# wtsi-svi/ReadServer

Hardware: AMD Instinct MI355X
Metric: 31-mer backward-search queries/sec on popBWT, counted as (query x shard) backward searches/s (higher is better)
Workload: dtype u64

## Files before the change

### readserver_amd/csrc/search_lines.hip

```cpp
#include <hip/hip_runtime.h>
#include <stdint.h>
#include <stdlib.h>
#include <string.h>

#include "kernels.h"
#include "line_format.h"
#include "rank_device.h"
#include "wave_lines.h"

namespace rsb {


__device__ __forceinline__ ulonglong2 start_record(const shard_view &ix, const uint64_t *pq, uint32_t k) {
    ulonglong2 rec;
    const uint64_t last = pq[(k - 1u) >> 5];
    if (view_uses_ktab(ix, k)) {
        const uint32_t T = ix.ktab_depth;
        const uint32_t off = 2u * (k - T);
        const uint32_t w0 = off >> 6, sh = off & 63u;
        uint64_t bits = (w0 == ((k - 1u) >> 5) ? last : pq[w0]) >> sh;
        if (sh + 2u * T > 64u) bits |= last << (64u - sh);
        const uint64_t e = ktab_entry(ix.ktab, ix.ktab_fmt, T, ix.ktab_stride, bits & ((1ull << (2u * T)) - 1ull));
        const uint32_t width = (uint32_t)(e >> COUNT_BITS);
        if (width != KTAB_WIDE && (e & COUNT_MASK) + width <= ix.n) {
// ... 101 lines not shown
    const uint32_t t = threadIdx.x;
    {
        const uint32_t v = t / nshards, s = t - v * nshards;
        if (v < V) {
            const shard_view &ix = shards[s];
            const bool tab = view_uses_ktab(ix, k);
            const uint32_t T = ix.ktab_depth, off = tab ? 2u * (k - T) : 0u;
            const uint64_t *ktab = ix.ktab;
            const uint32_t fmt = ix.ktab_fmt, stride = ix.ktab_stride;
            const uint64_t n = ix.n;
            uint8_t ok[INIT_U];
            uint64_t word[INIT_U], e[INIT_U];
#pragma unroll
            for (uint32_t u = 0; u < INIT_U; ++u) {
                const size_t q = q0 + (size_t)u * V + v;
                const bool in = q < Q;
                ok[u] = in ? valid[q] : (uint8_t)2;
                word[u] = in ? packed[q] : 0ull;
            }
#pragma unroll
            for (uint32_t u = 0; u < INIT_U; ++u)
                e[u] = (tab && ok[u] == 1) ? ktab_entry(ktab, fmt, T, stride, (word[u] >> off) & ((1ull << (2u * T)) - 1ull)) : ~0ull;
#pragma unroll
            for (uint32_t u = 0; u < INIT_U; ++u) {
                if (ok[u] == 2) continue;
                ulonglong2 rec;
                const uint32_t width = (uint32_t)(e[u] >> COUNT_BITS);
                if (ok[u] == 0) {
                    rec.x = INIT_INVALID;
                    rec.y = 0;
                } else if (tab && width != KTAB_WIDE && (e[u] & COUNT_MASK) + width <= n) {
                    rec.x = e[u] & COUNT_MASK;
                    rec.y = rec.x + width - 1ull;
                } else {
                    const uint32_t b = (uint32_t)((word[u] >> (2u * ((k - 1u) & 31u))) & 3u) + 1u;
                    rec.x = ix.C[b] | INIT_FALLBACK;
                    rec.y = ix.C[b] + ix.total[b] - 1ull;
                }
                tile[u][v * nshards + s] = rec;
            }
        }
    }
    __syncthreads();
    {
        const uint32_t s = t / V, v = t - s * V;
        if (s < nshards) {
#pragma unroll
            for (uint32_t u = 0; u < INIT_U; ++u) {
                const size_t q = q0 + (size_t)u * V + v;
                if (q < Q) init[(size_t)s * Q + q] = tile[u][v * nshards + s];
            }
        }
    }
}

__global__ void __launch_bounds__(256)
search_init_1mm_kernel(const shard_view *__restrict__ shards, uint32_t nshards, const uint64_t *__restrict__ vpacked,
                       const uint8_t *__restrict__ vvalid, size_t mv, uint32_t k, uint32_t wpq, uint32_t V,
                       const ulonglong2 *__restrict__ trace, uint32_t trace_n,
                       ulonglong2 *__restrict__ init) {
    const size_t t_ = (size_t)blockIdx.x * blockDim.x + threadIdx.x;
    if (t_ >= mv * nshards) return;
    const size_t i = t_ / nshards, s = t_ - i * nshards;
    ulonglong2 rec;
    if (vvalid[i] == 0) {
        rec.x = INIT_INVALID;
        rec.y = 0;
    } else {
        const size_t q = i / V;
        const uint32_t v = (uint32_t)(i - q * V);
        const uint32_t pos = v ? (v - 1u) / 3u : ~0u;
        if (pos < trace_n) {
            const ulonglong2 t = trace[(s * (mv / V) + q) * trace_n + pos];
            rec.x = (t.x & COUNT_MASK) | ((uint64_t)pos << COUNT_BITS) | INIT_EXPLICIT;
            rec.y = t.y;
        } else {
            rec = start_record(shards[s], vpacked + i * wpq, k);
        }
    }
    init[s * mv + i] = rec;
}

enum { WORK_STEPS = 0, WORK_OCC = 1, WORK_LINES = 2, WORK_KTAB = 3, WORK_PHASE0 = 4, WORK_PASSES = 10, WORK_HOPS = 11, WORK_SOLO = 12 };

template <bool COUNT_WORK, bool COUNTS_ONLY, bool LONGK, int ROLE>
__global__ void __launch_bounds__(64 * WG_WAVES, RSB_MIN_WGS_PER_CU)
search_lines_kernel(const shard_view *__restrict__ shards, uint32_t nshards, const uint64_t *__restrict__ packed,
                    const ulonglong2 *__restrict__ init, unsigned long long *__restrict__ next_query,
                    size_t Q, uint32_t k, uint32_t wpq,
                    uint64_t *__restrict__ out_lower, uint64_t *__restrict__ out_upper,
                    unsigned long long *__restrict__ work,
                    ulonglong2 *__restrict__ trace, uint32_t trace_n, uint32_t qchunk, uint32_t pairs) {
    __shared__ uint4 s_stage[WG_WAVES][64 * SLOT_U4];
    const uint32_t lane = threadIdx.x & 63u;
    const uint32_t wave = threadIdx.x >> 6;
    const uint32_t side = lane >> 5;
    uint4 *stage = s_stage[wave];
    const uint32_t stage_lds = __builtin_amdgcn_readfirstlane((uint32_t)(uintptr_t)(lds_void_ptr)stage);
    const uint32_t swz = lane & 7u;
    const lds_u32 *own_row = reinterpret_cast<const lds_u32 *>(stage + (lane & 7u) * 64u + (lane >> 3) * SLOT_U4);
#define MINE(d) (mine0 + (((((uint32_t)(d)) >> 2) ^ swz) << 2) + (((uint32_t)(d)) & 3u))

    unsigned long long w_steps = 0, w_occ = 0, w_lines = 0, w_hops = 0, w_ktab = 0;
    unsigned long long ph[6] = {0, 0, 0, 0, 0, 0}, stamp = 0, passes = 0;
#define STAMP(i)                                                        \
    if (COUNT_WORK) {                                                   \
        __builtin_amdgcn_sched_barrier(0);                              \
        const unsigned long long now_ = __builtin_amdgcn_s_memtime();   \
        asm volatile("s_waitcnt lgkmcnt(0)" ::: "memory");              \
        ph[i] += now_ - stamp;                                          \
        stamp = now_;                                                   \
        __builtin_amdgcn_sched_barrier(0);                              \
    }
    if (COUNT_WORK) stamp = __builtin_amdgcn_s_memtime();

    uint32_t sid = blockIdx.x % nshards;
    for (uint32_t visited = 0; visited < nshards; ++visited, sid = (sid + 1u == nshards) ? 0u : sid + 1u) {
        const shard_view *sv = shards + sid;
        const char *lines_bytes = reinterpret_cast<const char *>(sv->lines);
        const uint32_t S = sv->sp.S;
        const double inv = sv->sp.inv;
        const uint32_t nlines = (uint32_t)sv->nlines;
        const bool ktab = view_uses_ktab(*sv, k);
        const int j_table = ktab ? (int)(k - sv->ktab_depth) - 1 : (int)k - 2;
        const uint32_t w_table = j_table > 0 ? (uint32_t)j_table >> 5 : 0u;
        const ulonglong2 *init_s = init + (size_t)sid * Q;
        uint64_t *out_lo = out_lower + (size_t)sid * Q * (pairs ? 2u : 1u);
        uint64_t *out_up = (COUNTS_ONLY || pairs) ? nullptr : out_upper + (size_t)sid * Q;
        unsigned long long *pool = next_query + (size_t)sid * POOL_STRIDE;
        if (visited != 0u && __hip_atomic_load(pool, __ATOMIC_RELAXED, __HIP_MEMORY_SCOPE_AGENT) >= (unsigned long long)Q) continue;
        ulonglong2 *trace_s = trace ? trace + (size_t)sid * Q * trace_n : nullptr;
        unsigned long long *hit_map = pairs == 2u ? reinterpret_cast<unsigned long long *>(out_upper) + (size_t)sid * hit_map_words(Q) : nullptr;
        uint32_t ctab_lo, ctab_hi;
        {
            const uint64_t c1 = sv->C[1], c2 = sv->C[2], c3 = sv->C[3], c4 = sv->C[4];
            const uint32_t l3 = lane & 3u;
            const uint64_t cv = l3 == 0u ? c1 : l3 == 1u ? c2 : l3 == 2u ? c3 : c4;
            ctab_lo = (uint32_t)cv;
            ctab_hi = (uint32_t)(cv >> 32);
        }

        const uint32_t QCHUNK = qchunk;
        uint64_t pool_next = 0, pool_end = 0;
        bool drained = false;
        size_t q = 0;
        bool has_q = false;
        size_t nq = 0;
        bool has_n = false;
        ulonglong2 nrec = {0, 0};
        uint64_t nword = 0;
        int j = 0;
        uint64_t word = 0, lo = 0, hi = 0;
        bool ready = false;
        uint64_t occ_hold = 0, cacc = 0;
        uint32_t cont = 0, cblk = 0, cdw = 0, co = 0, tries = 0;

        for (;;) {
            bool done = false;
            if (!has_q && has_n) {
                has_q = true;
                has_n = false;
                q = nq;
                if (nrec.x & INIT_INVALID) {
                    lo = 1;
                    hi = 0;
                    j = -1;
// ... 209 lines not shown
                const uint64_t occL = side ? other : occ_hold;
                const uint64_t occU = side ? occ_hold : other;
                if (COUNT_WORK && side == 0u) w_steps += 1;
                lo = pb + occL;
                hi = pb + occU - 1ull;
                --j;
                done = (lo > hi) || (j < 0);
                ready = false;
            }
            if (got_n) {
                nrec = rec;
                nword = first_word;
                has_n = true;
            }
            if (alive && done) {
                if (trace && side == 0u) {
                    for (int jj = j < (int)trace_n ? j : (int)trace_n - 1; jj >= 0; --jj)
                        trace_s[q * trace_n + (uint32_t)jj] = make_ulonglong2(lo, hi);
                }
                if (side == 0u) {
                    if (COUNTS_ONLY) {
                        if (hi >= lo) out_lo[q] = hi - lo + 1ull;
                    } else if (pairs == 2u) {
                        if (lo <= hi) {
                            reinterpret_cast<ulonglong2 *>(out_lo)[q] = make_ulonglong2(lo, hi);
                            atomicOr(hit_map + (q >> 6), 1ull << (q & 63u));
                        }
                    } else if (pairs) {
#ifdef RSB_NT_RESULTS
                        __builtin_nontemporal_store(lo, &out_lo[2 * q]);
                        __builtin_nontemporal_store(hi, &out_lo[2 * q + 1]);
#else
                        reinterpret_cast<ulonglong2 *>(out_lo)[q] = make_ulonglong2(lo, hi);
#endif
                    } else {
                        out_lo[q] = lo;
                        out_up[q] = hi;
                    }
                }
                has_q = false;
            }
            STAMP(5)
            if (COUNT_WORK) ++passes;
        }
    }
    if (COUNT_WORK) {
        if (lane == 0u) {
            for (int i = 0; i < 6; ++i) atomicAdd(&work[WORK_PHASE0 + i], ph[i]);
            atomicAdd(&work[WORK_PASSES], passes);
        }
        if (w_steps) atomicAdd(&work[WORK_STEPS], w_steps);
        if (w_occ) atomicAdd(&work[WORK_OCC], w_occ);
        if (w_lines) atomicAdd(&work[WORK_LINES], w_lines);
        if (w_ktab) atomicAdd(&work[WORK_KTAB], w_ktab);
        if (w_hops) atomicAdd(&work[WORK_HOPS], w_hops);
    }
#undef MINE
#undef STAMP
}

}
#include "search_solo.h"
namespace rsb {

static int search_kernel_choice() {
    static const int choice = [] {
        const char *e = getenv("RSBWT_SEARCH_KERNEL");
        if (e && !strcmp(e, "pair")) return 0;
        if (e && !strcmp(e, "solo")) return 1;
        return 2;
    }();
    return choice;
}

template <bool CW, bool CO>
static void launch_solo(int grid, hipStream_t stream, const shard_view *shards, uint32_t nshards, const uint64_t *pk,
                        const ulonglong2 *init, const uint8_t *valid, unsigned long long *ctr, size_t Q, uint32_t k, uint32_t wpq,
                        uint64_t *lo, uint64_t *up, unsigned long long *work, ulonglong2 *trace, uint32_t trace_n,
                        uint32_t pairs, bool fused) {
    uint32_t qchunk = 1024;
    while (qchunk > 64u && (size_t)qchunk * (size_t)grid * WG_WAVES * 4u > Q * nshards) qchunk >>= 1;
    static const bool no_staged = getenv("RSBWT_NO_STAGED_RESULTS") != nullptr;
    const bool staged = !CO && pairs != 2u && !no_staged;
    const uint32_t pa = pairs | (staged ? SOLO_STAGED_RESULTS : 0u);
    const size_t dyn = staged ? SOLO_RESULTS_LDS : 0u;
    if (fused)
        hipLaunchKernelGGL((search_solo_kernel<CW, CO, false, true>), dim3(grid), dim3(64 * WG_WAVES), dyn, stream, shards, nshards,
                           pk, init, valid, ctr, Q, k, wpq, lo, up, work, trace, trace_n, qchunk, pa);
    else if (wpq > 1)
        hipLaunchKernelGGL((search_solo_kernel<CW, CO, true>), dim3(grid), dim3(64 * WG_WAVES), dyn, stream, shards, nshards,
                           pk, init, valid, ctr, Q, k, wpq, lo, up, work, trace, trace_n, qchunk, pa);
    else
        hipLaunchKernelGGL((search_solo_kernel<CW, CO, false>), dim3(grid), dim3(64 * WG_WAVES), dyn, stream, shards, nshards,
                           pk, init, valid, ctr, Q, k, wpq, lo, up, work, trace, trace_n, qchunk, pa);
}

template <bool CW, bool CO>
static void launch_k(int grid, hipStream_t stream, const shard_view *shards, uint32_t nshards, const uint64_t *pk,
                     const ulonglong2 *init, unsigned long long *ctr, size_t Q, uint32_t k, uint32_t wpq,
                     uint64_t *lo, uint64_t *up, unsigned long long *work, ulonglong2 *trace, uint32_t trace_n,
                     uint32_t pairs) {
    uint32_t qchunk = 1024;
    while (qchunk > 32u && (size_t)qchunk * (size_t)grid * WG_WAVES * 4u > Q * nshards) qchunk >>= 1;
    if (wpq > 1)
        hipLaunchKernelGGL((search_lines_kernel<CW, CO, true, 0>), dim3(grid), dim3(64 * WG_WAVES), 0, stream, shards, nshards,
                           pk, init, ctr, Q, k, wpq, lo, up, work, trace, trace_n, qchunk, pairs);
    else
        hipLaunchKernelGGL((search_lines_kernel<CW, CO, false, 0>), dim3(grid), dim3(64 * WG_WAVES), 0, stream, shards, nshards,
                           pk, init, ctr, Q, k, wpq, lo, up, work, trace, trace_n, qchunk, pairs);
}

static void launch_init(const shard_view *d_shards, uint32_t nshards, const uint64_t *pk, const uint8_t *vd, size_t Q, uint32_t k,
                        uint32_t wpq, ulonglong2 *init, hipStream_t stream) {
    static const bool untiled = getenv("RSBWT_INIT_UNTILED") != nullptr;
    static const bool one_per_thread = getenv("RSBWT_INIT_ONE_PER_THREAD") != nullptr;
    if (nshards >= 2u && nshards <= 256u && !untiled && wpq == 1u && !one_per_thread) {
        const uint32_t V = 256u / nshards;
        hipLaunchKernelGGL(search_init_tiled4_kernel, dim3((unsigned)((Q + (size_t)V * INIT_U - 1) / ((size_t)V * INIT_U))), dim3(256), 0, stream,
                           d_shards, nshards, pk, vd, Q, k, V, init);
    } else if (nshards >= 2u && nshards <= 256u && !untiled) {
        const uint32_t V = 256u / nshards;
        hipLaunchKernelGGL(search_init_tiled_kernel, dim3((unsigned)((Q + V - 1) / V)), dim3(256), 0, stream, d_shards, nshards, pk, vd, Q,
                           k, wpq, V, init);
    } else {
        const size_t nrec = Q * nshards;
        hipLaunchKernelGGL(search_init_kernel, dim3((unsigned)((nrec + 255) / 256)), dim3(256), 0, stream, d_shards, nshards, pk, vd, Q, k,
                           wpq, init);
    }
}

hipError_t launch_search_init_var(const shard_view *d_shards, uint32_t nshards, const void *d_packed, const void *d_valid,
                                  const void *d_len, size_t Q, uint32_t wpq, void *d_init, hipStream_t stream) {
    if (Q == 0 || nshards == 0) return hipSuccess;
    const size_t nrec = Q * nshards;
    hipLaunchKernelGGL(search_init_var_kernel, dim3((unsigned)((nrec + 255) / 256)), dim3(256), 0, stream, d_shards, nshards,
                       (const uint64_t *)d_packed, (const uint8_t *)d_valid, (const uint32_t *)d_len, Q, wpq, (ulonglong2 *)d_init);
    return hipGetLastError();
}

hipError_t launch_search_init(const shard_view *d_shards, uint32_t nshards, const void *d_packed, const void *d_valid, size_t Q,
                              uint32_t k, void *d_init, hipStream_t stream) {
    if (Q == 0 || nshards == 0) return hipSuccess;
    const uint32_t wpq = (k + 31u) / 32u ? (k + 31u) / 32u : 1u;
    launch_init(d_shards, nshards, (const uint64_t *)d_packed, (const uint8_t *)d_valid, Q, k, wpq, (ulonglong2 *)d_init, stream);
    return hipGetLastError();
}

hipError_t launch_search(scratch_cache &scratch, const shard_view *d_shards, uint32_t nshards, const void *d_packed,
                         const void *d_valid, size_t Q, uint32_t k, void *d_lower, void *d_upper, bool counts_only,
                         unsigned long long *d_work, int num_cus, hipStream_t stream, hipEvent_t ev0, hipEvent_t ev1,
                         const search_extra *extra) {
    if (Q == 0 || nshards == 0) return hipSuccess;
    if (extra && extra->table_build && nshards != 1) return hipErrorInvalidValue;
    const bool hit_list = extra && extra->d_hit_bits && !counts_only;
    const uint32_t pairs = hit_list ? 2u : (extra && extra->pairs && !counts_only) ? 1u : 0u;
    ulonglong2 *trace = extra ? (ulonglong2 *)extra->d_trace_out : nullptr;
    const uint32_t trace_n = extra ? extra->trace_n : 0u;
    const uint32_t wpq = (k + 31u) / 32u ? (k + 31u) / 32u : 1u;
    const bool table_build = extra && extra->table_build;
    const int choice = search_kernel_choice();
    size_t g = 0;
    static const int wgs_per_cu = [] {
        const char *e = getenv("RSBWT_WAVE_WGS_PER_CU");
        const int v = e ? atoi(e) : 0;
        return v > 0 ? v : RSB_MIN_WGS_PER_CU;
    }();
    static const size_t spare_wgs = [] {
// ... 183 lines not shown
```

### readserver_amd/csrc/search_solo.h

```cpp
#ifndef RSBWT_SEARCH_SOLO_H
#define RSBWT_SEARCH_SOLO_H

namespace rsb {

constexpr uint64_t WL_DEAD = 1ull << 63;
constexpr uint32_t SOLO_STAGED_RESULTS = 4u;
constexpr uint32_t SOLO_RESULTS_LDS = WG_WAVES * 2048u;
constexpr uint32_t RES_BUFS = 15u;

#ifndef RSB_WALK1MM_WGS_PER_CU
#define RSB_WALK1MM_WGS_PER_CU 3
#endif
template <bool COUNT_WORK, bool COUNTS_ONLY, bool LONGK, bool FUSED = false, bool WL = false, bool WALK = false>
__global__ void __launch_bounds__(64 * WG_WAVES, WALK ? RSB_WALK1MM_WGS_PER_CU : RSB_MIN_WGS_PER_CU)
search_solo_kernel(const shard_view *__restrict__ shards, uint32_t nshards, const uint64_t *__restrict__ packed,
                   const ulonglong2 *__restrict__ init, const uint8_t *__restrict__ valid,
                   unsigned long long *__restrict__ next_query,
                   size_t Q, uint32_t k, uint32_t wpq,
                   uint64_t *__restrict__ out_lower, uint64_t *__restrict__ out_upper,
                   unsigned long long *__restrict__ work,
                   ulonglong2 *__restrict__ trace, uint32_t trace_n, uint32_t qchunk, uint32_t pairs_arg,
                   const unsigned long long *__restrict__ wl_counts = nullptr, size_t wl_cap = 0, size_t wl_implicit = 0) {
    __shared__ uint4 s_stage[WG_WAVES][64 * SLOT_U4];
    extern __shared__ uint4 s_results[];
    const uint32_t lane = threadIdx.x & 63u;
    const uint32_t wave = threadIdx.x >> 6;
    uint4 *stage = s_stage[wave];
    const uint32_t stage_lds = __builtin_amdgcn_readfirstlane((uint32_t)(uintptr_t)(lds_void_ptr)stage);
    const uint32_t swz = lane & 7u;
    const uint32_t pairs = pairs_arg & 3u;
    constexpr bool CAN_STAGE = !COUNTS_ONLY && !WL && !WALK;
    const bool stage_out = CAN_STAGE && (pairs_arg & SOLO_STAGED_RESULTS) != 0u && pairs != 2u && Q < (1ull << 34);
    uint4 *results = s_results + wave * 128u;
    uint32_t *res_state = reinterpret_cast<uint32_t *>(results + RES_BUFS * 8u);
    const lds_u32 *mine0 = reinterpret_cast<const lds_u32 *>(stage + (lane & 7u) * 64u + (lane >> 3) * SLOT_U4);
#define SOLO_MINE(d) (mine0 + (((((uint32_t)(d)) >> 2) ^ swz) << 2) + (((uint32_t)(d)) & 3u))

    unsigned long long w_steps = 0, w_occ = 0, w_lines = 0, w_hops = 0, w_ktab = 0, passes = 0;
    unsigned long long w_surv = 0, w_unstepped = 0;

    uint32_t sid = blockIdx.x % nshards;
    for (uint32_t visited = 0; visited < nshards; ++visited, sid = (sid + 1u == nshards) ? 0u : sid + 1u) {
        const shard_view *sv = shards + sid;
        const char *lines_bytes = reinterpret_cast<const char *>(sv->lines);
        const uint32_t S = sv->sp.S;
        const double inv = sv->sp.inv;
        const uint32_t nlines = (uint32_t)sv->nlines;
        const bool ktab = view_uses_ktab(*sv, k);
        const int j_table = ktab ? (int)(k - sv->ktab_depth) - 1 : (int)k - 2;
        const uint32_t w_table = j_table > 0 ? (uint32_t)j_table >> 5 : 0u;
        const ulonglong2 *init_s = WL ? init + (size_t)sid * wl_cap * 2u : init + (size_t)sid * Q;
        const size_t Qs = WALK ? Q : WL ? wl_implicit + (size_t)(wl_counts[(size_t)sid * WL_COUNT_STRIDE] < wl_cap ? wl_counts[(size_t)sid * WL_COUNT_STRIDE] : wl_cap) : Q;
        const uint32_t wl_tn = trace_n, wl_per = WL ? 3u * (k - trace_n) : 1u;
        const size_t walk_V = 3u * (size_t)k + 1u, walk_mv = Q * walk_V;
        ulonglong2 *walk_wl = WALK ? const_cast<ulonglong2 *>(init) + (size_t)sid * wl_cap * 2u : nullptr;
        unsigned long long *walk_count = WALK ? const_cast<unsigned long long *>(wl_counts) + (size_t)sid * WL_COUNT_STRIDE : nullptr;
        uint64_t *out_lo = WALK ? out_lower + (size_t)sid * walk_mv * 2u : out_lower + (size_t)sid * Q * (pairs ? 2u : 1u);
        uint64_t *out_up = (COUNTS_ONLY || pairs) ? nullptr : out_upper + (size_t)sid * Q;
        unsigned long long *pool = next_query + (size_t)sid * POOL_STRIDE;
        if (visited != 0u && __hip_atomic_load(pool, __ATOMIC_RELAXED, __HIP_MEMORY_SCOPE_AGENT) >= (unsigned long long)Qs) continue;
        ulonglong2 *trace_s = (trace && !WL) ? trace + (size_t)sid * Q * trace_n : nullptr;
        const uint64_t *wl_pre = (WL && trace) ? reinterpret_cast<const uint64_t *>(trace) + (size_t)sid * wl_implicit : nullptr;
        unsigned long long *hit_map = pairs == 2u ? reinterpret_cast<unsigned long long *>(out_upper) + (size_t)sid * hit_map_words(WALK ? walk_mv : Q) : nullptr;
        uint32_t ctab_lo, ctab_hi;
        {
            const uint64_t c1 = sv->C[1], c2 = sv->C[2], c3 = sv->C[3], c4 = sv->C[4];
            const uint32_t l3 = lane & 3u;
            const uint64_t cv = l3 == 0u ? c1 : l3 == 1u ? c2 : l3 == 2u ? c3 : c4;
            ctab_lo = (uint32_t)cv;
            ctab_hi = (uint32_t)(cv >> 32);
        }

        const uint64_t *__restrict__ ktab_p = sv->ktab;
        const uint32_t ktab_T = sv->ktab_depth, ktab_stride = sv->ktab_stride, ktab_fmt = sv->ktab_fmt;
        const uint64_t ix_n = sv->n;
        const uint64_t sc1 = sv->C[1], sc2 = sv->C[2], sc3 = sv->C[3], sc4 = sv->C[4];
        const uint64_t st1 = sv->total[1], st2 = sv->total[2], st3 = sv->total[3], st4 = sv->total[4];

        const uint32_t QCHUNK = qchunk;
        if (CAN_STAGE && stage_out && lane < RES_BUFS) {
            res_state[2u * lane] = ~0u;
            res_state[2u * lane + 1u] = 0u;
        }
        uint64_t pool_next = 0, pool_end = 0;
        bool drained = false;
        size_t q = 0;
        bool has_q = false;
        size_t nq = 0;
        bool has_n = false;
        ulonglong2 nrec = {0, 0};
        uint64_t nword = 0;
        uint32_t nstage = 0;
        bool nimp = false;
        int j = 0;
        uint64_t word = 0, lo = 0, hi = 0;
        uint32_t sub = 0;
        uint64_t occL = 0, cacc = 0;
        uint32_t cont = 0, cblk = 0, cdw = 0, co = 0, tries = 0, w = 0;
        uint64_t altL0 = 0, altL1 = 0, altL2 = 0, altU0 = 0, altU1 = 0, altU2 = 0;
        bool alt_ok = true;

        for (;;) {
            bool done = false;
            bool last_in = false;
            if (FUSED && !has_q && has_n && nstage == 2u) {
                const uint64_t e = nrec.x;
                const uint32_t width = (uint32_t)(e >> COUNT_BITS);
                if (nrec.y == 0ull) {
                    nrec.x = INIT_INVALID;
                } else if (width != KTAB_WIDE && (e & COUNT_MASK) + width <= ix_n) {
                    nrec.x = e & COUNT_MASK;
                    nrec.y = nrec.x + width - 1ull;
                } else {
                    const uint32_t bl = (uint32_t)((nword >> (2u * ((k - 1u) & 31u))) & 3u);
                    const uint64_t cb = bl == 0u ? sc1 : bl == 1u ? sc2 : bl == 2u ? sc3 : sc4;
                    const uint64_t tb = bl == 0u ? st1 : bl == 1u ? st2 : bl == 2u ? st3 : st4;
                    nrec.x = cb | INIT_FALLBACK;
                    nrec.y = cb + tb - 1ull;
                }
            }
            if (WL && !has_q && has_n && nstage == 2u) {
                has_q = true;
// ... 9 lines not shown
                    const uint32_t width = (uint32_t)(e >> COUNT_BITS);
                    bool tabulated = false;
                    if (width != KTAB_WIDE && (e & COUNT_MASK) + width <= ix_n) {
                        lo = e & COUNT_MASK;
                        hi = lo + width - 1ull;
                        j = (int)wl_tn - 1;
                        tabulated = true;
                    } else {
                        const uint32_t bl = (uint32_t)((nword >> (2u * ((k - 1u) & 31u))) & 3u);
                        const uint64_t cb = bl == 0u ? sc1 : bl == 1u ? sc2 : bl == 2u ? sc3 : sc4;
                        const uint64_t tb = bl == 0u ? st1 : bl == 1u ? st2 : bl == 2u ? st3 : st4;
                        lo = cb;
                        hi = cb + tb - 1ull;
                        j = (int)k - 2;
                    }
                    done = (nrec.y & 0xFFull) == 0ull || (tabulated && lo > hi) || j < 0;
                } else {
                    q = nq;
                    lo = nrec.x & COUNT_MASK;
                    hi = nrec.y;
                    j = (int)((nrec.x >> COUNT_BITS) & 0xFFFFull);
                    done = (nrec.x & WL_DEAD) != 0ull || lo > hi;
                }
                if (done) { lo = 1; hi = 0; }
            }
            if (!WL && !has_q && has_n && (!FUSED || nstage == 2u)) {
                has_q = true;
                has_n = false;
                q = nq;
                sub = 0;
                cont = 0;
                if (nrec.x & INIT_INVALID) {
                    lo = 1;
                    hi = 0;
                    j = -1;
                    done = true;
                } else if (nrec.x & INIT_EXPLICIT) {
                    lo = nrec.x & COUNT_MASK;
                    hi = nrec.y;
                    j = (int)((nrec.x >> COUNT_BITS) & 0xFFFFull) - ((nrec.x & INIT_VAR) ? 1 : 0);
                    word = nword;
                    done = j < 0 || ((nrec.x & INIT_NOCHECK) == 0ull && lo > hi);
                    if (LONGK) {
                        if (!done && ((uint32_t)j >> 5) != w_table) word = packed[q * wpq + ((uint32_t)j >> 5)];
                    }
                } else {
                    const bool fallback = !ktab || (nrec.x & INIT_FALLBACK) != 0ull;
                    lo = nrec.x & COUNT_MASK;
                    hi = nrec.y;
                    j = fallback ? (int)k - 2 : j_table;
                    word = nword;
                    if (COUNT_WORK && !fallback) w_ktab += 1;
                    done = (j < 0) || (!fallback && lo > hi);
                    if (LONGK) {
                        if (!done && ((uint32_t)j >> 5) != w_table) word = packed[q * wpq + ((uint32_t)j >> 5)];
                    }
                }
            }
            if (pool_next >= pool_end && !drained) {
                unsigned long long c = 0;
                if (lane == 0u) c = atomicAdd(pool, (unsigned long long)QCHUNK);
                c = ((unsigned long long)__builtin_amdgcn_readfirstlane((uint32_t)(c >> 32)) << 32) |
                    __builtin_amdgcn_readfirstlane((uint32_t)c);
                pool_next = c;
                pool_end = c + QCHUNK < Qs ? c + QCHUNK : Qs;
                if (c >= Qs) { drained = true; pool_next = pool_end = 0; }
            }
            bool got_n = false;
            {
                const uint64_t want_mask = __builtin_amdgcn_ballot_w64(!has_n);
                const uint32_t before = (uint32_t)__builtin_popcountll(want_mask & ((1ull << lane) - 1ull));
                const uint64_t mine = pool_next + before;
                if (!has_n && mine < pool_end) {
                    nq = (size_t)mine;
                    got_n = true;
                }
                const uint64_t taken = pool_next + (uint32_t)__builtin_popcountll(want_mask);
                const uint64_t r0 = pool_next;
                pool_next = taken < pool_end ? taken : pool_end;
                if (CAN_STAGE && stage_out && pool_next > r0) {
                    const uint64_t first = (r0 + 7ull) & ~7ull;
                    if (first < pool_next) {
                        const uint32_t ga = (uint32_t)(first >> 3), gb = (uint32_t)((pool_next - 1ull) >> 3) + 1u;
                        const uint32_t ga15 = ga % RES_BUFS;
                        if (lane < RES_BUFS) {
                            const uint32_t d = lane >= ga15 ? lane - ga15 : lane + RES_BUFS - ga15;
                            const uint32_t g = ga + d;
                            if (g < gb && res_state[2u * lane + 1u] == 0u) {
                                const uint64_t q0 = (uint64_t)g << 3;
                                res_state[2u * lane] = g;
                                res_state[2u * lane + 1u] = (uint32_t)((q0 + 8ull < pool_end ? q0 + 8ull : pool_end) - q0);
                            }
                        }
                    }
                }
            }
            if (__builtin_amdgcn_ballot_w64(has_q || got_n || ((FUSED || WL) && has_n)) == 0ull) {
                if (drained) break;
                continue;
            }
            ulonglong2 rec = {0, 0};
            uint64_t first_word = 0;
            const bool stage_b = (FUSED || WL) && has_n && nstage == 1u;
            uint64_t entry = 0;
            uint64_t wl_index = 0, vword = 0;
            bool imp = false;
            if (WL) {
                if (got_n) {
                    imp = nq < wl_implicit;
                    if (imp) {
                        const uint32_t i32 = (uint32_t)nq, q_ = i32 / wl_per, r_ = i32 - q_ * wl_per;
                        first_word = packed[q_];
                        rec.y = (uint64_t)valid[q_] | ((uint64_t)r_ << 8) | ((uint64_t)q_ << 32);
                    } else {
                        const size_t slot = nq - wl_implicit;
                        rec = init_s[2u * slot];
                        const ulonglong2 r2 = init_s[2u * slot + 1u];
                        wl_index = r2.x;
                        first_word = r2.y;
                    }
                }
                if (stage_b) {
                    const uint32_t r_ = (uint32_t)(nrec.y >> 8) & 0xFFu;
                    const uint32_t pr = (r_ * 171u) >> 9, d_ = r_ - 3u * pr, p_ = wl_tn + pr;
                    const uint32_t orig = (uint32_t)((nword >> (2u * p_)) & 3u);
                    const uint32_t alt = d_ < orig ? d_ : d_ + 1u;
                    vword = nword ^ ((uint64_t)(orig ^ alt) << (2u * p_));
                    const uint64_t code = (vword >> (2u * wl_tn)) & ((1ull << (2u * ktab_T)) - 1ull);
                    entry = wl_pre ? wl_pre[nq] : ktab_entry(ktab_p, ktab_fmt, ktab_T, ktab_stride, code);
                }
            } else if (FUSED) {
                if (got_n) {
                    rec.y = valid[nq];
                    first_word = packed[nq];
                }
                if (stage_b) {
                    const uint64_t code = (nword >> (2u * (k - ktab_T))) & ((1ull << (2u * ktab_T)) - 1ull);
                    entry = ktab_entry(ktab_p, ktab_fmt, ktab_T, ktab_stride, code);
                }
            } else if (got_n) {
                rec = init_s[nq];
                first_word = packed[nq * wpq + w_table];
            }
            const bool alive = has_q;
            const bool stepping = alive && !done;
            const bool fresh = stepping && cont == 0u;

            uint32_t b = 1, line = 0, o = 0;
            if (stepping) {
                if (LONGK) {
                    if (fresh && sub == 0u && (j & 31) == 31) word = packed[q * wpq + ((uint32_t)j >> 5)];
                }
                b = (uint32_t)((word >> (2u * ((uint32_t)j & 31u))) & 3u) + 1u;
            }
            bool no_fetch = false;
            if (fresh) {
                if (sub == 0u) {
                    if (WALK) {
                        alt_ok = true;
                        altL0 = altL1 = altL2 = altU0 = altU1 = altU2 = 0;
                    }
                    if (trace_s && (uint32_t)j < trace_n) trace_s[q * trace_n + (uint32_t)j] = make_ulonglong2(lo, hi);
                    if (lo == 0ull) {
                        occL = 0;
                        sub = 1u;
                    }
                }
                const uint64_t p = sub ? hi : lo - 1ull;
                if (p == ~0ull) {
                    no_fetch = true;
                } else {
                    uint32_t pin;
                    w = fast_window(p, S, inv, pin);
                    line = w + (w >> GROUP_SHIFT);
                    o = pin + 1u;
                    if (line >= nlines) line = 0;
                    if (COUNT_WORK) w_occ += 1;
// ... 144 lines not shown
                const staged_line Lrow = {mine0, swz};
                const line_head hh = {s1, s2, s3, span, 0u};
#pragma unroll 1
                for (uint32_t ev = 0; ev < 2u; ++ev) {
                    const bool want = ev == 0u ? ev1 : (second && (uint32_t)j < trace_n);
                    if (__builtin_amdgcn_ballot_w64(want) == 0ull) continue;
                    uint64_t t3[3];
                    staged_occ_alts(Lrow, hh, want ? (ev == 0u ? oe_here : oh) : 1u, b - 1u, t3);
                    if (want) {
                        if (ev == 0u && ev1_is_L) { altL0 = t3[0]; altL1 = t3[1]; altL2 = t3[2]; }
                        else { altU0 = t3[0]; altU1 = t3[1]; altU2 = t3[2]; }
                    }
                }
                const bool emit = step_done && (uint32_t)j < trace_n;
                if (__builtin_amdgcn_ballot_w64(emit) != 0ull) {
                    const uint32_t orig = b - 1u;
                    uint64_t nlo[3], nhi[3], masks[3];
                    bool enq[3];
#pragma unroll
                    for (uint32_t d = 0; d < 3u; ++d) {
                        const uint32_t alt = d < orig ? d : d + 1u;
                        const uint64_t cb = ((uint64_t)(uint32_t)__builtin_amdgcn_ds_bpermute((int)(alt << 2), (int)ctab_hi) << 32) |
                                            (uint32_t)__builtin_amdgcn_ds_bpermute((int)(alt << 2), (int)ctab_lo);
                        nlo[d] = cb + (d == 0u ? altL0 : d == 1u ? altL1 : altL2);
                        nhi[d] = cb + (d == 0u ? altU0 : d == 1u ? altU1 : altU2) - 1ull;
                        const bool stepped_live = emit && alt_ok && nlo[d] <= nhi[d];
                        const bool final_hit = stepped_live && j == 0;
                        enq[d] = (stepped_live && j != 0) || (emit && !alt_ok);
                        if (final_hit) {
                            const size_t canon = q * walk_V + 1u + 3u * (uint32_t)j + d;
                            reinterpret_cast<ulonglong2 *>(out_lo)[canon] = make_ulonglong2(nlo[d], nhi[d]);
                            atomicOr(hit_map + (canon >> 6), 1ull << (canon & 63u));
                        }
                        masks[d] = __builtin_amdgcn_ballot_w64(enq[d]);
                        if (COUNT_WORK) {
                            w_surv += __builtin_popcountll(__builtin_amdgcn_ballot_w64((enq[d] && alt_ok) || final_hit));
                            w_unstepped += __builtin_popcountll(__builtin_amdgcn_ballot_w64(enq[d] && !alt_ok));
                        }
                    }
                    if (COUNT_WORK && emit) w_steps += 3;
                    const uint32_t n0 = (uint32_t)__builtin_popcountll(masks[0]), n1 = (uint32_t)__builtin_popcountll(masks[1]);
                    const uint32_t total = n0 + n1 + (uint32_t)__builtin_popcountll(masks[2]);
                    if (total != 0u) {
                        unsigned long long wbase = 0;
                        if (lane == 0u) wbase = atomicAdd(walk_count, (unsigned long long)total);
                        wbase = ((unsigned long long)(uint32_t)__builtin_amdgcn_readfirstlane((int)(uint32_t)(wbase >> 32)) << 32) |
                                (uint32_t)__builtin_amdgcn_readfirstlane((int)(uint32_t)wbase);
                        const uint64_t lt = (1ull << lane) - 1ull;
#pragma unroll
                        for (uint32_t d = 0; d < 3u; ++d) {
                            if (!enq[d]) continue;
                            const size_t slot = (size_t)wbase + (d >= 1u ? n0 : 0u) + (d >= 2u ? n1 : 0u) + (size_t)__builtin_popcountll(masks[d] & lt);
                            if (slot >= wl_cap) continue;
                            const uint32_t alt = d < orig ? d : d + 1u;
                            const uint64_t vword = word ^ ((uint64_t)(orig ^ alt) << (2u * (uint32_t)j));
                            const uint64_t canon = (uint64_t)q * walk_V + 1ull + 3ull * (uint32_t)j + d;
                            if (!alt_ok) wl_store(walk_wl, slot, lo, (uint32_t)j, hi, canon, vword);
                            else wl_store(walk_wl, slot, nlo[d], (uint32_t)j - 1u, nhi[d], canon, vword);
                        }
                    }
                }
            }
            if (step_done) {
                if (COUNT_WORK) w_steps += 1;
                lo = pb + occL;
                hi = pb + occU - 1ull;
                --j;
                done = (lo > hi) || (j < 0);
                sub = 0;
            }
            if ((FUSED || WL) && stage_b) {
                nrec.x = entry;
                nstage = 2u;
                if (WL) nword = vword;
            }
            if (got_n) {
                nrec = rec;
                nword = first_word;
                has_n = true;
                nstage = (WL && !imp) ? 2u : 1u;
                nimp = imp;
                if (WL && !imp) nq = (size_t)wl_index;
            }
            if (alive && done) {
                if (trace_s) {
                    for (int jj = j < (int)trace_n ? j : (int)trace_n - 1; jj >= 0; --jj)
                        trace_s[q * trace_n + (uint32_t)jj] = make_ulonglong2(lo, hi);
                }
                if (COUNTS_ONLY) {
                    if (hi >= lo) out_lo[q] = hi - lo + 1ull;
                } else if (pairs == 2u) {
                    if (lo <= hi) {
                        const size_t qi = WALK ? q * walk_V : q;
                        reinterpret_cast<ulonglong2 *>(out_lo)[qi] = make_ulonglong2(lo, hi);
                        atomicOr(hit_map + (qi >> 6), 1ull << (qi & 63u));
                    }
                } else {
                    const uint32_t g32 = (uint32_t)(q >> 3), rb = g32 % RES_BUFS;
                    if (CAN_STAGE && stage_out && res_state[2u * rb] == g32) {
                        results[rb * 8u + ((uint32_t)q & 7u)] = make_uint4((uint32_t)lo, (uint32_t)(lo >> 32), (uint32_t)hi, (uint32_t)(hi >> 32));
                        last_in = atomicSub(&res_state[2u * rb + 1u], 1u) == 1u;
                    } else if (pairs) {
                        reinterpret_cast<ulonglong2 *>(out_lo)[q] = make_ulonglong2(lo, hi);
                    } else {
                        out_lo[q] = lo;
                        out_up[q] = hi;
                    }
                }
                has_q = false;
            }
            if (CAN_STAGE && stage_out) {
                uint64_t fm = __builtin_amdgcn_ballot_w64(last_in);
                while (fm != 0ull) {
                    const int src = __builtin_ctzll(fm);
                    fm &= fm - 1ull;
                    const uint32_t g = (uint32_t)__builtin_amdgcn_readlane((int)(uint32_t)(q >> 3), src), bsel = g % RES_BUFS;
                    const size_t qq = ((size_t)g << 3) + lane;
                    if (lane < 8u && qq < Qs) {
                        const uint4 v = results[bsel * 8u + lane];
                        const uint64_t vlo = ((uint64_t)v.y << 32) | v.x, vhi = ((uint64_t)v.w << 32) | v.z;
                        if (pairs) {
                            reinterpret_cast<ulonglong2 *>(out_lo)[qq] = make_ulonglong2(vlo, vhi);
                        } else {
                            out_lo[qq] = vlo;
                            out_up[qq] = vhi;
                        }
                    }
                }
            }
            if (COUNT_WORK) ++passes;
        }
    }
    if (COUNT_WORK) {
        if (lane == 0u) atomicAdd(&work[WORK_PASSES], passes);
        if (threadIdx.x == 0u && blockIdx.x == 0u) work[WORK_SOLO] = 1ull;
        if (w_steps) atomicAdd(&work[WORK_STEPS], w_steps);
        if (w_occ) atomicAdd(&work[WORK_OCC], w_occ);
        if (w_lines) atomicAdd(&work[WORK_LINES], w_lines);
        if (w_ktab) atomicAdd(&work[WORK_KTAB], w_ktab);
        if (w_hops) atomicAdd(&work[WORK_HOPS], w_hops);
        if (WALK && lane == 0u) {
            atomicAdd(&work[13], w_surv);
            atomicAdd(&work[14], w_unstepped);
        }
    }
#undef SOLO_MINE
}

}
#endif
```

Baseline: 4.181 billion.

## Compress staged solo results to 8-byte slots and add more LDS buffers

Staged result slots in LDS shrink from 16 bytes (lo,hi) to 8 bytes (40-bit lo plus 24-bit width). Within the same 2 KB per wave this raises the number of result buffers from 15 to 28, so more query groups can be staged and written out as coalesced 8-lane stores instead of falling back to scattered direct stores. Results that do not fit (wide intervals or large lo) are escaped and stored directly by the owning lane. Wave-level LDS release/acquire fences are added around the staging handoffs, and an optional counter of unstaged results is added for diagnostics.

```diff
diff --git a/readserver_amd/csrc/search_lines.hip b/readserver_amd/csrc/search_lines.hip
--- a/readserver_amd/csrc/search_lines.hip
+++ b/readserver_amd/csrc/search_lines.hip
@@ -207,6 +207,7 @@
 }
 
 enum { WORK_STEPS = 0, WORK_OCC = 1, WORK_LINES = 2, WORK_KTAB = 3, WORK_PHASE0 = 4, WORK_PASSES = 10, WORK_HOPS = 11, WORK_SOLO = 12 };
+enum { WORK_UNSTAGED = 15 };
 
 template <bool COUNT_WORK, bool COUNTS_ONLY, bool LONGK, int ROLE>
 __global__ void __launch_bounds__(64 * WG_WAVES, RSB_MIN_WGS_PER_CU)
@@ -582,7 +583,8 @@
     while (qchunk > 64u && (size_t)qchunk * (size_t)grid * WG_WAVES * 4u > Q * nshards) qchunk >>= 1;
     static const bool no_staged = getenv("RSBWT_NO_STAGED_RESULTS") != nullptr;
     const bool staged = !CO && pairs != 2u && !no_staged;
-    const uint32_t pa = pairs | (staged ? SOLO_STAGED_RESULTS : 0u);
+    static const bool count_unstaged = getenv("RSBWT_COUNT_UNSTAGED") != nullptr;
+    const uint32_t pa = pairs | (staged ? SOLO_STAGED_RESULTS : 0u) | (CW && count_unstaged ? SOLO_COUNT_UNSTAGED : 0u);
     const size_t dyn = staged ? SOLO_RESULTS_LDS : 0u;
     if (fused)
         hipLaunchKernelGGL((search_solo_kernel<CW, CO, false, true>), dim3(grid), dim3(64 * WG_WAVES), dyn, stream, shards, nshards,
diff --git a/readserver_amd/csrc/search_solo.h b/readserver_amd/csrc/search_solo.h
--- a/readserver_amd/csrc/search_solo.h
+++ b/readserver_amd/csrc/search_solo.h
@@ -5,8 +5,23 @@
 
 constexpr uint64_t WL_DEAD = 1ull << 63;
 constexpr uint32_t SOLO_STAGED_RESULTS = 4u;
-constexpr uint32_t SOLO_RESULTS_LDS = WG_WAVES * 2048u;
-constexpr uint32_t RES_BUFS = 15u;
+constexpr uint32_t SOLO_COUNT_UNSTAGED = 8u;
+constexpr uint32_t RES_WAVE_LDS = 2048u;
+constexpr uint32_t SOLO_RESULTS_LDS = WG_WAVES * RES_WAVE_LDS;
+constexpr uint32_t RES_SLOT_BYTES = 8u;
+constexpr uint32_t RES_STATE_BYTES = 8u;
+constexpr uint32_t RES_BUFS = RES_WAVE_LDS / (8u * RES_SLOT_BYTES + RES_STATE_BYTES);
+static_assert(RES_BUFS * (8u * RES_SLOT_BYTES + RES_STATE_BYTES) <= RES_WAVE_LDS, "a wave's buffers and their state fit its 2 KB");
+static_assert(RES_WAVE_LDS == 2048u && RES_BUFS == 28u, "2 KB per wave: with the line slots a CU's 160 KB at four workgroups");
+static_assert(RES_BUFS >= 9u && RES_BUFS <= 64u, "a lane per buffer claims; at most 9 groups begin among a pass's 64 draws");
+constexpr uint32_t RES_WIDTH_BITS = 24u;
+constexpr uint32_t RES_ESCAPED = (1u << RES_WIDTH_BITS) - 1u;
+
+__device__ __forceinline__ void solo_lds_handoff() {
+    __builtin_amdgcn_fence(__ATOMIC_RELEASE, "wavefront", "local");
+    __builtin_amdgcn_wave_barrier();
+    __builtin_amdgcn_fence(__ATOMIC_ACQUIRE, "wavefront", "local");
+}
 
 #ifndef RSB_WALK1MM_WGS_PER_CU
 #define RSB_WALK1MM_WGS_PER_CU 3
@@ -31,13 +46,15 @@
     const uint32_t pairs = pairs_arg & 3u;
     constexpr bool CAN_STAGE = !COUNTS_ONLY && !WL && !WALK;
     const bool stage_out = CAN_STAGE && (pairs_arg & SOLO_STAGED_RESULTS) != 0u && pairs != 2u && Q < (1ull << 34);
-    uint4 *results = s_results + wave * 128u;
+    uint2 *results = reinterpret_cast<uint2 *>(s_results + wave * (RES_WAVE_LDS / 16u));
     uint32_t *res_state = reinterpret_cast<uint32_t *>(results + RES_BUFS * 8u);
+    const bool count_unstaged = COUNT_WORK && (pairs_arg & SOLO_COUNT_UNSTAGED) != 0u;
     const lds_u32 *mine0 = reinterpret_cast<const lds_u32 *>(stage + (lane & 7u) * 64u + (lane >> 3) * SLOT_U4);
 #define SOLO_MINE(d) (mine0 + (((((uint32_t)(d)) >> 2) ^ swz) << 2) + (((uint32_t)(d)) & 3u))
 
     unsigned long long w_steps = 0, w_occ = 0, w_lines = 0, w_hops = 0, w_ktab = 0, passes = 0;
     unsigned long long w_surv = 0, w_unstepped = 0;
+    unsigned long long w_unstaged = 0;
 
     uint32_t sid = blockIdx.x % nshards;
     for (uint32_t visited = 0; visited < nshards; ++visited, sid = (sid + 1u == nshards) ? 0u : sid + 1u) {
@@ -213,9 +230,9 @@
                     const uint64_t first = (r0 + 7ull) & ~7ull;
                     if (first < pool_next) {
                         const uint32_t ga = (uint32_t)(first >> 3), gb = (uint32_t)((pool_next - 1ull) >> 3) + 1u;
-                        const uint32_t ga15 = ga % RES_BUFS;
+                        const uint32_t gam = ga % RES_BUFS;
                         if (lane < RES_BUFS) {
-                            const uint32_t d = lane >= ga15 ? lane - ga15 : lane + RES_BUFS - ga15;
+                            const uint32_t d = lane >= gam ? lane - gam : lane + RES_BUFS - gam;
                             const uint32_t g = ga + d;
                             if (g < gb && res_state[2u * lane + 1u] == 0u) {
                                 const uint64_t q0 = (uint64_t)g << 3;
@@ -224,6 +241,7 @@
                             }
                         }
                     }
+                    solo_lds_handoff();
                 }
             }
             if (__builtin_amdgcn_ballot_w64(has_q || got_n || ((FUSED || WL) && has_n)) == 0ull) {
@@ -534,6 +552,7 @@
                 nimp = imp;
                 if (WL && !imp) nq = (size_t)wl_index;
             }
+            if (CAN_STAGE && stage_out) solo_lds_handoff();
             if (alive && done) {
                 if (trace_s) {
                     for (int jj = j < (int)trace_n ? j : (int)trace_n - 1; jj >= 0; --jj)
@@ -549,19 +568,28 @@
                     }
                 } else {
                     const uint32_t g32 = (uint32_t)(q >> 3), rb = g32 % RES_BUFS;
+                    bool own_store = true;
                     if (CAN_STAGE && stage_out && res_state[2u * rb] == g32) {
-                        results[rb * 8u + ((uint32_t)q & 7u)] = make_uint4((uint32_t)lo, (uint32_t)(lo >> 32), (uint32_t)hi, (uint32_t)(hi >> 32));
+                        const uint64_t width = hi - lo + 1ull;
+                        own_store = width >= (uint64_t)RES_ESCAPED || (lo >> COUNT_BITS) != 0ull;
+                        results[rb * 8u + ((uint32_t)q & 7u)] =
+                            own_store ? make_uint2(0u, RES_ESCAPED << 8) : make_uint2((uint32_t)lo, (uint32_t)(lo >> 32) | ((uint32_t)width << 8));
                         last_in = atomicSub(&res_state[2u * rb + 1u], 1u) == 1u;
-                    } else if (pairs) {
-                        reinterpret_cast<ulonglong2 *>(out_lo)[q] = make_ulonglong2(lo, hi);
-                    } else {
-                        out_lo[q] = lo;
-                        out_up[q] = hi;
+                    }
+                    if (own_store) {
+                        if (pairs) {
+                            reinterpret_cast<ulonglong2 *>(out_lo)[q] = make_ulonglong2(lo, hi);
+                        } else {
+                            out_lo[q] = lo;
+                            out_up[q] = hi;
+                        }
+                        if (count_unstaged) w_unstaged += 1;
                     }
                 }
                 has_q = false;
             }
             if (CAN_STAGE && stage_out) {
+                solo_lds_handoff();
                 uint64_t fm = __builtin_amdgcn_ballot_w64(last_in);
                 while (fm != 0ull) {
                     const int src = __builtin_ctzll(fm);
@@ -569,9 +597,11 @@
                     const uint32_t g = (uint32_t)__builtin_amdgcn_readlane((int)(uint32_t)(q >> 3), src), bsel = g % RES_BUFS;
                     const size_t qq = ((size_t)g << 3) + lane;
                     if (lane < 8u && qq < Qs) {
-                        const uint4 v = results[bsel * 8u + lane];
-                        const uint64_t vlo = ((uint64_t)v.y << 32) | v.x, vhi = ((uint64_t)v.w << 32) | v.z;
-                        if (pairs) {
+                        const uint2 v = results[bsel * 8u + lane];
+                        const uint32_t width = v.y >> 8;
+                        const uint64_t vlo = ((uint64_t)(v.y & 0xFFu) << 32) | v.x, vhi = vlo + width - 1ull;
+                        if (width == RES_ESCAPED) {
+                        } else if (pairs) {
                             reinterpret_cast<ulonglong2 *>(out_lo)[qq] = make_ulonglong2(vlo, vhi);
                         } else {
                             out_lo[qq] = vlo;
@@ -591,6 +621,7 @@
         if (w_lines) atomicAdd(&work[WORK_LINES], w_lines);
         if (w_ktab) atomicAdd(&work[WORK_KTAB], w_ktab);
         if (w_hops) atomicAdd(&work[WORK_HOPS], w_hops);
+        if (w_unstaged) atomicAdd(&work[WORK_UNSTAGED], w_unstaged);
         if (WALK && lane == 0u) {
             atomicAdd(&work[13], w_surv);
             atomicAdd(&work[14], w_unstepped);
```

Result: faster. 4.248 billion, median of 6 (+1.6%).
